# moldyn/Clustering

Hardware: AMD Instinct MI355X
Metric: frame-pairs/s (density pop+nn) (higher is better)
Workload: dtype f32 (Gram form on two fp16 pieces per coordinate on the f16 MFMA pipe, f32 accumulate, as a classifier with a guard band; undecided pairs re-checked in canonical f32)

## Files before the change

clustering_amd/csrc/dc_mfma.hip:

```cpp
#include "dc_mfma_kernels.hpp"
#include "dc_against.hpp"
#include "dc_against_nn.hpp"

#include <algorithm>
#include <cstring>
#include <atomic>
#include <mutex>

#ifndef DC_STEP_MASK
#define DC_STEP_MASK 0xFFFFu
#endif

namespace dc {

namespace {

#include "dc_mfma32.hpp"

__global__ void colsum_kernel(const float* __restrict__ coords, uint32_t n_rows, uint32_t D,
                              double* __restrict__ sums) {
  __shared__ double part[kMaxCols];
  if (threadIdx.x < (uint32_t)kMaxCols) part[threadIdx.x] = 0.0;
  __syncthreads();
  const uint32_t nthreads = gridDim.x * blockDim.x;
// ... 871 lines not shown
    auto env = [](const char* name) -> const char* {
      const char* v = getenv(name);
      return (v && v[0]) ? v : nullptr;
    };
    auto one_of_124 = [](const char* v, int dflt) {
      const int k = v ? atoi(v) : dflt;
      return (k == 1 || k == 2 || k == 4) ? k : dflt;
    };
    SweepSwitches w;
    const char* v;
    if ((v = env("DC_POP_SYM"))) w.pop_sym = v[0] != '0';
    if ((v = env("DC_POP_SHARED"))) w.pop_shared = atoi(v);
    if ((v = env("DC_NN_SHARED"))) w.nn_shared = atoi(v);
    w.waves_per_group = one_of_124(env("DC_WAVES_PER_GROUP"), 0);
    if ((v = env("DC_NN_COOP"))) w.nn_coop = atoi(v);
    if ((v = env("DC_WAVE_TARGET"))) w.wave_target = (uint32_t)atoi(v);
    if ((v = env("DC_SHARE_FLOOR"))) w.share_floor = (uint32_t)atoi(v);
    if ((v = env("DC_POP_COMPONENTS"))) w.components = v[0] != '0';
    w.pop_cell_frames = (v = env("DC_POP_CELL_FRAMES")) ? (float)atof(v) : kPopCellFrames;
    w.nn_cell_frames = (v = env("DC_NN_CELL_FRAMES")) ? (float)atof(v) : kNnCellFrames;
    if ((v = env("DC_NN_FE_BITS"))) w.nn_fe_bits = atoi(v);
    w.mfma32_wpb = (uint32_t)one_of_124(env("DC_MFMA32_WPB"), 1);
    if ((v = env("DC_MFMA32_CHUNKS"))) w.mfma32_chunks = (uint32_t)atoi(v);
    return w;
  }();
  return sw;
}

static float cell_frames(bool nn) { return nn ? sweep_switches().nn_cell_frames : sweep_switches().pop_cell_frames; }
static float nn_cell_frames() { return cell_frames(true); }
// ... 319 lines not shown

static int order_own_queries(const PrunedWs& W, const Layout& L, const QueryPlan& Q, const float* d_coords, uint32_t n_rows,
                             uint32_t n_cols, unsigned fine_bits, uint32_t i_from, uint32_t i_to, hipStream_t stream) {
  char* p = W.p;
  const dim3 blk(256);
  const uint32_t kb_q = std::min<uint32_t>((std::max(Q.n_q, 32u * Q.T_q) + 255) / 256, 1024u);
  hipLaunchKernelGGL(order_key_kernel, dim3(kb_q), blk, 0, stream, d_coords, n_cols, W.hdr, (const uint32_t*)W.comp,
                     (uint32_t)fine_bits, i_from, i_to, W.sort.keys_in, W.sort.vals_in, n_rows, (const float*)nullptr, 0u, W.cnt_tab, 0,
                     W.perm_q, W.tile_comp_q, 32u * Q.T_q);
  hipLaunchKernelGGL(order_meta_kernel, dim3(1), dim3(1024), 0, stream, W.hdr, W.comp, (const uint32_t*)W.cnt_tab, kb_q, W.start_q,
                     W.range_q, W.base_q, Q.n_q, Q.group_rows, 0, 0.0f, n_cols);
  const SortRemap remap{W.start_q, W.base_q, (uint32_t)kMaxComp, W.tile_comp_q};
  if (int rc = W.sort.run(W.perm_q, Q.n_q, stream, fine_bits, &remap)) return rc;
  hipLaunchKernelGGL(order_rows2_kernel, dim3((32 * Q.T_q + 255) / 256), blk, order_rows_smem_set(n_cols), stream, d_coords, n_cols,
                     L.NM, (const uint32_t*)W.perm_q, Q.T_q, (float*)nullptr, (float4*)(p + L.off_box_q), (const float*)nullptr,
                     (float*)nullptr, (uint32_t*)nullptr, (float2*)nullptr, (const uint32_t*)W.tile_comp_q, W.origins, W.hdr,
                     (uint4*)nullptr, 0, (float*)nullptr, (uint4*)(p + L.off_img_q), (float*)(p + L.off_norm_q), 1u,
                     QSeg{1u, 0u, 1u}, (unsigned long long*)nullptr, (uint32_t*)nullptr, 0u);
  return 0;
}

static void pop_pruned_one(const PopPlan& plan, const float* d_coords, uint32_t n_rows, uint32_t n_cols,
                           const QuerySel& qs, const Rad2& rad2, int n_rad, uint32_t* d_pops, void* d_ws,
                           const EdgeSink* sink_in, hipStream_t stream, float r2_scale, bool prep, bool comp_clean) {
  const Layout L = make_layout(n_rows, n_cols);
  const PrunedWs W = pruned_ws(d_ws, L, n_rows);
  char* p = W.p;
  const dim3 blk(256), grid_n((n_rows + 255) / 256);
  const QueryPlan Q = query_plan(qs, n_rows, plan.group_tiles);
  const uint32_t T_r = Q.T_r;
  const float r_max = sqrtf(fmaxf(r2_scale, 0.0f)) * 1.0001f;
// ... 11 lines not shown
  if (prep) {
    const uint32_t cookie = data_cookie(d_coords, n_rows, n_cols);
    if (!comp_clean) (void)hipMemsetAsync(W.comp, 0, sizeof(uint32_t) * kCompWords, stream);
    hipLaunchKernelGGL(fine_mark_kernel, grid_n, blk, 0, stream, d_coords, n_rows, n_cols, (const uint32_t*)W.hdr, r_conn,
                       W.comp);
    hipLaunchKernelGGL(components_kernel, dim3(1), dim3(1024), components_smem(), stream, (const uint32_t*)W.hdr,
                       (const float*)(p + kHdrMeans), n_cols, r_conn, n_rows, kPopCellFrames, fine_bits, W.comp,
                       components_off() ? 1 : 0, r_max, cookie, (const double*)(p + L.fixed_end), cell_frames(false));
    if (order_refs(W, Q, d_coords, n_rows, n_cols, fine_bits, nullptr, 0u, fine_bits, fmaxf(r2_scale, 0.0f), plan.shift_steps,
                   stream))
      return;
    {
      const bool ref_queries = Q.q_mode != kQueryOwnOrder;
      hipLaunchKernelGGL(order_rows2_kernel, dim3((32 * T_r + 255) / 256), blk, order_rows_smem_set(n_cols), stream, d_coords, n_cols,
                         L.NM, (const uint32_t*)W.perm_p, T_r, (float*)(p + L.off_coords_p), (float4*)(p + L.off_box_p),
                         (const float*)nullptr, (float*)nullptr, (uint32_t*)nullptr, (float2*)nullptr, (const uint32_t*)W.tile_comp,
                         W.origins, W.hdr, (uint4*)(p + L.off_img_p), 0, (float*)(p + L.off_norm_p),
                         ref_queries ? (uint4*)(p + L.off_img_q) : (uint4*)nullptr, (float*)nullptr, plan.group_tiles, Q.q_seg,
                         (unsigned long long*)(W.comp + kCompHash), pos_clean ? (uint32_t*)(p + L.off_pq) : (uint32_t*)nullptr, 1u);
    }
    if (sink_in && sink_in->best) {
      hipLaunchKernelGGL(gather_u32_kernel, dim3((32 * T_r + 255) / 256), blk, 0, stream, sink_in->comp,
                         (const uint32_t*)W.perm_p, 32u * T_r, W.sort.keys_in);
      hipLaunchKernelGGL(gather_u32_kernel, dim3((32 * T_r + 255) / 256), blk, 0, stream, sink_in->rank,
                         (const uint32_t*)W.perm_p, 32u * T_r, W.sort.keys_out);
    }
    if (Q.q_mode == kQueryOwnOrder &&
        order_own_queries(W, L, Q, d_coords, n_rows, n_cols, fine_bits, qs.i_from, qs.i_to, stream))
      return;
  }
  const uint32_t n_pos_q = 32u * ((Q.q_mode == kQueryOwnOrder) ? Q.T_q : T_r);
// ... 256 lines not shown
  if (reuse_components) {
  } else {
    hipLaunchKernelGGL(fe_key_kernel, dim3(std::min<uint32_t>(grid_n.x, 256u)), blk, 0, stream, d_fe, n_rows, (uint32_t*)nullptr,
                       (uint32_t*)nullptr, W.hdr);
    if (!comp_clean) (void)hipMemsetAsync(W.comp, 0, sizeof(uint32_t) * kCompWords, stream);
    hipLaunchKernelGGL(fine_mark_kernel, grid_n, blk, 0, stream, d_coords, n_rows, n_cols, (const uint32_t*)W.hdr, r_conn, W.comp);
    hipLaunchKernelGGL(components_kernel, dim3(1), dim3(1024), components_smem(), stream, (const uint32_t*)W.hdr,
                       (const float*)(p + kHdrMeans), n_cols, r_conn, n_rows, kNnCellFrames, fine_bits, W.comp,
                       components_off() ? 1 : 0, 0.0f, cookie, (const double*)(p + L.fixed_end), cell_frames(true));
  }
  if (order_refs(W, Q, d_coords, n_rows, n_cols, fine_bits, d_fe, fe_bits, fine_bits + fe_bits, -1.0f ,
                 0, stream))
    return;
  const float* coords_p = (const float*)(p + L.off_coords_p);
  {
    hipLaunchKernelGGL(order_rows2_kernel, dim3((32 * T_r + 255) / 256), blk, order_rows_smem_set(n_cols), stream, d_coords, n_cols,
                       L.NM, (const uint32_t*)W.perm_p, T_r, (float*)(p + L.off_coords_p), (float4*)(p + L.off_box_p), d_fe,
                       (float*)(p + L.off_fe_s), (uint32_t*)(p + L.off_invpos), (float2*)(p + L.off_ferange_p),
                       (const uint32_t*)W.tile_comp, W.origins, W.hdr, (uint4*)(p + L.off_img_p), 2, (float*)(p + L.off_norm_p),
                       own ? (uint4*)nullptr : (uint4*)(p + L.off_img_q), (float*)nullptr, plan.group_tiles, Q.q_seg,
                       (unsigned long long*)(W.comp + kCompHash), (uint32_t*)nullptr, 0u);
  }
  if (own && order_own_queries(W, L, Q, d_coords, n_rows, n_cols, fine_bits, qs.i_from, qs.i_to, stream))
    return;
  const uint32_t n_pos_q = 32u * (own ? Q.T_q : T_r);
  switch (nm_for((int)n_cols)) {
#define X(SV)                                                                                   \
  case SV:                                                                                      \
    if ((DC_STEP_MASK >> (SV - 1)) & 1u)                                                        \
      nn_pruned_step_##SV(plan, d_coords, n_rows, n_cols, d_fe, d_ws, T_r, n_pos_q, Q.q_mode, Q.q_seg, -1.0f, \
                          d_nn_idx, d_nn_d2, d_hd_idx, d_hd_d2, stream);                        \
    break;
    DC_FOR_EACH_S(X)
// ... 489 lines not shown
```

clustering_amd/csrc/dc_mfma.hpp:

```cpp
#pragma once
#include "dc_common.hpp"

namespace dc {

struct EdgeSink {
  uint2* edges;
  unsigned long long* count;
  unsigned long long capacity;
  const uint32_t* comp;
  const uint32_t* rank;
  unsigned long long* best;
};
enum SinkMode { kSinkNone = 0, kSinkPairs = 1, kSinkMinEdge = 2 };

struct SweepSwitches {
  bool pop_sym = true;
  int pop_shared = -1;
  int nn_shared = -1;
  int waves_per_group = 0;
  int nn_coop = -1;
  uint32_t wave_target = 0;
  uint32_t share_floor = 0;
  bool components = true;
  float pop_cell_frames = 0.0f;
  float nn_cell_frames = 0.0f;
  int nn_fe_bits = -1;
  uint32_t mfma32_wpb = 1;
  uint32_t mfma32_chunks = 0;
};
const SweepSwitches& sweep_switches();

enum PopForm {
  kPopWave,
  kPopWaveSym,
  kPopPairs,
// ... 141 lines not shown
```

clustering_amd/csrc/dc_mfma_kernels.hpp:

```cpp
#pragma once
#include "dc_mfma.hpp"
#include "dc_credit.hpp"

#include <assert.h>
#include <float.h>
#include <math.h>
#include <stdlib.h>

#include <type_traits>

namespace dc {

namespace {

typedef float f32x16 __attribute__((ext_vector_type(16)));
typedef short s16x8 __attribute__((ext_vector_type(8)));

constexpr int kMaxCols = 64;
constexpr int kConstSlots = 2;
constexpr int kPieceGroups = 3;
constexpr int nm_for(int n_cols) { return (kPieceGroups * n_cols + kConstSlots + 15) / 16; }
constexpr int kMaxMfma = nm_for(kMaxCols);
constexpr size_t kHdrBytes = 1024;
constexpr size_t kHdrSums = 256;
// ... 23 lines not shown
constexpr size_t kCompAdj = kCompRange + 2 * kCompRangeStride;
constexpr size_t kCompBox = kCompAdj + 2 * (size_t)kMaxComp;
constexpr size_t kCompBitmap = kCompBox + 4 * (size_t)kMaxComp;
constexpr size_t kCompBitmapWords = (size_t)kCoarseCells * kFineSub * kFineSub / 4;
constexpr size_t kCompBase = kCompBitmap + kCompBitmapWords;
constexpr size_t kCompHash = ((kCompBase + 2 * ((size_t)kMaxComp + 1)) + 1) & ~(size_t)1;
constexpr size_t kCompWords = kCompHash + 2 * 64;

struct Layout {
  uint32_t T, NM;
  uint32_t Tp;
  size_t off_img, off_img_b, off_norm, off_img_s, off_norm_s, off_fe_s, off_perm, off_invpos, off_pq,
      off_keys_in, off_keys_out, off_vals_in,
      off_img_p, off_norm_p, off_perm_p, off_box_p, off_img_q, off_norm_q, off_perm_q, off_box_q,
      off_ferange_p,
      off_coords_p,
      off_merge64,
      off_box_t,
      off_comp,
      off_tile_comp, off_tile_comp_q,
      fixed_end;
};

inline size_t align256(size_t x) { return (x + 255) & ~(size_t)255; }

inline Layout make_layout(size_t n_rows, size_t n_cols) {
  Layout L;
  L.T = (uint32_t)((n_rows + 31) / 32);
  L.NM = (uint32_t)nm_for((int)n_cols);
  L.Tp = L.T + kPadTiles;
  const size_t img_bytes = (size_t)16 * 64 * (size_t)L.Tp * L.NM;
  const size_t row_bytes = align256(sizeof(float) * 32 * (size_t)L.Tp);
  L.off_comp = kHdrBytes;
// ... 6 lines not shown
  L.off_perm = L.off_fe_s + row_bytes;
  L.off_invpos = L.off_perm + row_bytes;
  L.off_pq = L.off_invpos + row_bytes;
  L.off_keys_in = L.off_pq + row_bytes;
  L.off_keys_out = L.off_keys_in + row_bytes;
  L.off_vals_in = L.off_keys_out + row_bytes;
  L.off_img_p = L.off_vals_in + row_bytes;
  L.off_norm_p = align256(L.off_img_p + img_bytes);
  L.off_perm_p = L.off_norm_p + row_bytes;
  L.off_box_p = L.off_perm_p + row_bytes;
  L.off_img_q = align256(L.off_box_p + sizeof(float) * 4 * (size_t)L.Tp);
  L.off_norm_q = align256(L.off_img_q + img_bytes);
  L.off_perm_q = L.off_norm_q + row_bytes;
  L.off_box_q = L.off_perm_q + row_bytes;
  L.off_ferange_p = align256(L.off_box_q + sizeof(float) * 4 * (size_t)L.Tp);
  L.off_coords_p = align256(L.off_ferange_p + sizeof(float) * 2 * (size_t)L.Tp);
  L.off_merge64 = align256(L.off_coords_p + sizeof(float) * 32 * (size_t)L.Tp * n_cols);
  L.off_box_t = align256(L.off_merge64 + sizeof(unsigned long long) * 2 * n_rows);
  L.off_tile_comp = align256(L.off_box_t + sizeof(float) * 4 * ((size_t)L.Tp + L.Tp / 32 + 64));
  L.off_tile_comp_q = align256(L.off_tile_comp + sizeof(uint32_t) * (size_t)L.Tp);
  L.fixed_end = align256(L.off_tile_comp_q + sizeof(uint32_t) * (size_t)L.Tp);
  return L;
}

struct Ptrs {
  const uint32_t* hdr;
  const double* sums;
  const uint4* img;
  const uint4* img_b;
  const float* norms;
  const uint4* img_s;
  const float* norms_s;
  const float* fe_s;
  const uint32_t* perm;
// ... 1555 lines not shown
__device__ __forceinline__ void load_tile_folded(const uint4* __restrict__ img, uint32_t t, int lane, s16x8 (&a)[NM]) {
  const uint4* ip = img + (size_t)t * (NM * 64) + lane;
#pragma unroll
  for (int m = 0; m < NM; ++m) {
    const uint4 v = ip[m * 64];
    a[m] = __builtin_bit_cast(s16x8, v);
  }
}

template <int NM, int TQ, bool COOP = false>
__global__ __launch_bounds__(COOP ? 512 : 256, COOP ? 1 : 2) void nn_pruned_kernel(
    const float* __restrict__ coords, uint32_t n_rows, uint32_t n_cols,
    const float* __restrict__ fe, const uint4* __restrict__ img_r,
    const float* __restrict__ norms_r, const uint32_t* __restrict__ perm_r,
    const float4* __restrict__ box_r, const float4* __restrict__ box_t,
    const float2* __restrict__ ferange_r,
    const float* __restrict__ fe_c, const float* __restrict__ coords_c,
    const uint32_t* __restrict__ invpos_r, uint32_t T,
    const uint4* __restrict__ img_q, const float* __restrict__ norms_q,
    const uint32_t* __restrict__ perm_q, const float4* __restrict__ box_q, uint32_t n_q, QSeg q_seg,
    int full_range, float cell2,
    const uint32_t* __restrict__ hdr, unsigned long long* __restrict__ chain_counter,
    unsigned long long* __restrict__ merge64, uint32_t* __restrict__ nn_idx,
    float* __restrict__ nn_d2, uint32_t* __restrict__ hd_idx, float* __restrict__ hd_d2, CompView CV) {
  extern __shared__ __attribute__((aligned(16))) float nn_dyn_lds[];
  if (hdr[1] != 0) return;
  const int lane = threadIdx.x & 63, h = lane >> 5, c = lane & 31;
  const int wib = threadIdx.x >> 6;
  const uint32_t wpb = blockDim.x >> 6;
  uint32_t* lists_all = reinterpret_cast<uint32_t*>(nn_dyn_lds);
// ... 240 lines not shown
    own_hi = (uint32_t)__builtin_amdgcn_readfirstlane((int)own_hi);
  }
  const float fe_floor = fkey_inv(~hdr[12]);
  auto flush = [&]() {
    nn_wave_flush(cand, qn, qrows, best64, TQ * 32, coords_c, perm_r, n_cols, lane);
    qn = 0;
  };
  uint32_t chains = 0, visited = 0;
  uint32_t chains_on = 0;
  const uint32_t t_lo = comp_lo, t_hi = min(comp_hi, T);
  const uint32_t u_lo = (t_lo > chunk) ? (t_lo - chunk + n_chunks - 1) / n_chunks : 0u;
  const uint32_t U = max((t_hi > chunk) ? (t_hi - chunk + n_chunks - 1) / n_chunks : 0u, u_lo);
  cell2 = comp_cell * comp_cell;
  const uint32_t U_stride = (T + n_chunks - 1) / n_chunks;
  const float dgx = gbox.y - gbox.x, dgy = gbox.w - gbox.z;
  float r2_lo = -1.0f;
  float r2_hi = fmaxf(dgx * dgx + dgy * dgy, cell2);
  if (!(r2_hi > 0.0f)) r2_hi = FLT_MIN;
  for (;;) {
    for (uint32_t base = u_lo; base < U; base += kListCap) {
      uint32_t cnt = 0;
      const uint32_t lim = min(U - base, (uint32_t)kListCap);
      auto tile_of = [&](uint32_t u) { return chunk + u * n_chunks; };
      const float4* box_s = box_t + (size_t)chunk * U_stride;
      float4 rb_next = ((uint32_t)lane < lim) ? box_s[base + lane]
                                              : make_float4(INFINITY, -INFINITY, INFINITY, -INFINITY);
      for (uint32_t k = 0; k < lim; k += 64) {
        const uint32_t t = tile_of(base + k + lane);
        const float4 rb = rb_next;
        if (k + 64 + lane < lim) rb_next = box_s[base + k + 64 + lane];
        bool ok = false;
        if (k + lane < lim) {
          const float g2 = box_gap2(gbox, rb);
          ok = (g2 < r2_hi) & (g2 >= r2_lo);
        }
        const uint64_t m = __builtin_amdgcn_ballot_w64(ok);
        if (ok) list[cnt + __builtin_amdgcn_mbcnt_hi((uint32_t)(m >> 32), __builtin_amdgcn_mbcnt_lo((uint32_t)m, 0))] = t;
        cnt += (uint32_t)__builtin_popcountll(m);
      }
      if (cnt == 0) continue;
      visited += cnt;
      uint32_t cN = 0, cH = 0;
      if constexpr (kNnEarly<NM>) {
        constexpr int kSteps = kListCap / 64;
        uint32_t e[kSteps], cls[kSteps];
        float2 fr[kSteps];
#pragma unroll
        for (int j = 0; j < kSteps; ++j) {
// ... 366 lines not shown
  const uint32_t waves = (tiles + tq - 1) / tq;
  return (waves + 3) / 4;
}

template <int S, SweepMode M>
void pop_dispatch(const SweepArgs& X, uint32_t n_cols, uint32_t i_from, uint32_t i_to, const Rad2& rad2, uint32_t* pops,
                  hipStream_t s) {
  constexpr int kTQ = tq_full_for<S>;
  const dim3 grid(grid_for(i_from, i_to, kTQ)), block(256);
  sweep_timer_mark(0, true, s);
  hipLaunchKernelGGL((pop_mfma_kernel<S, 1, kTQ, M>), grid, block, 0, s, X, n_cols, i_from, i_to, rad2, 1, pops);
  sweep_timer_mark(0, false, s);
}

__global__ void box_by_share_kernel(const float4* __restrict__ box_r, uint32_t T, uint32_t n_chunks,
                                    float4* __restrict__ box_t) {
  const uint32_t t = blockIdx.x * blockDim.x + threadIdx.x;
  if (t >= T) return;
  const uint32_t stride = (T + n_chunks - 1) / n_chunks;
  box_t[(size_t)(t % n_chunks) * stride + t / n_chunks] = box_r[t];
}

struct NnPrunedArgs {
  const uint4* img_r;
  const float* norms_r;
  const uint32_t* perm_r;
  const float4* box_r;
  float4* box_t;
  const float2* ferange_r;
  const float* fe_c;
  const float* coords_c;
  const uint32_t* invpos_r;
  const uint4* img_q;
  const float* norms_q;
  const uint32_t* perm_q;
  const float4* box_q;
  unsigned long long* merge64;
  uint32_t n_q;
  QSeg q_seg;
  int full_range;
  float cell2;
  const uint32_t* tile_comp_q;
  const uint32_t* comp;
// ... 83 lines not shown
  if (sw.share_floor) share_floor = sw.share_floor;
  const uint32_t waves = (tiles + tq - 1) / tq;
  uint32_t r = waves >= target ? 1u : (target + waves - 1) / waves;
  const uint32_t by_share = ref_tiles / share_floor;
  const uint32_t cap = by_share < 64u ? by_share : 64u;
  r = r > cap ? cap : r;
  return r < 1u ? 1u : r;
}

template <class F>
void timed_launch(int kind, hipStream_t s, F&& launch) {
  sweep_timer_mark(kind, true, s);
  launch();
  sweep_timer_mark(kind, false, s);
}
inline void nn_shares_begin(const NnPrunedArgs& A, uint32_t n_rows, uint32_t T, uint32_t n_chunks, hipStream_t s) {
  if (n_chunks > 1)
    hipLaunchKernelGGL(nn_merge_fill_kernel, dim3((2 * n_rows + 255) / 256), dim3(256), 0, s, A.merge64, n_rows);
  hipLaunchKernelGGL(box_by_share_kernel, dim3((T + 255) / 256), dim3(256), 0, s, A.box_r, T, n_chunks, A.box_t);
}
inline void nn_shares_end(const NnPrunedArgs& A, uint32_t n_rows, uint32_t n_chunks, uint32_t group_tiles,
                          uint32_t* nn_idx, float* nn_d2, uint32_t* hd_idx, float* hd_d2, hipStream_t s) {
  if (n_chunks <= 1) return;
  if (A.full_range)
    hipLaunchKernelGGL(nn_merge_unpack_rows_kernel, dim3((n_rows + 255) / 256), dim3(256), 0, s,
                       (const unsigned long long*)A.merge64, A.invpos_r, n_rows, group_tiles, A.q_seg, nn_idx, nn_d2,
                       hd_idx, hd_d2);
  else
    hipLaunchKernelGGL(nn_merge_unpack_kernel, dim3((A.n_q + 255) / 256), dim3(256), 0, s,
                       (const unsigned long long*)A.merge64, A.perm_q, A.n_q, n_rows, group_tiles, A.q_seg, nn_idx,
                       nn_d2, hd_idx, hd_d2);
}

template <int S>
void nn_pruned_dispatch(const NnPlan& pl, const float* coords, uint32_t n_rows, uint32_t n_cols, const float* fe,
                        const NnPrunedArgs& A, uint32_t T, const uint32_t* hdr,
                        unsigned long long* chain_counter, uint32_t* nn_idx, float* nn_d2,
                        uint32_t* hd_idx, float* hd_d2, hipStream_t s) {
  assert(nn_form_built(pl.form, S));
  if (A.n_q == 0) return;
  const CompView CV{A.tile_comp_q, A.comp + kCompRange, 32u * T, A.comp};
  if (pl.form == kNnShared) {
    if constexpr (nn_form_built(kNnShared, S)) {
      constexpr int TQV = tq_wave(S);
      assert(pl.tq == (uint32_t)TQV);
      const uint32_t groups = seg_groups(((A.n_q + 31) / 32 + 4 * TQV - 1) / (4 * TQV), A.q_seg);
      if (groups == 0) return;
      const uint32_t n_chunks = pick_chunks(groups * 4 * TQV, TQV, kNnWaveTarget, T, kNnShareFloor, (size_t)S * 1024 + 128);
      const size_t smem = (size_t)kRing * (S * 64 + kNnRingExtra) * 16 + sizeof(uint32_t) * 4 * (TQV * kQueueCap * 64 + TQV * 32);
      nn_shares_begin(A, n_rows, T, n_chunks, s);
      constexpr int kNbMax = kNnCoarseMax<S>;
      constexpr int kNbMin = (S > 1) ? nn_coarse_for((16 * (S - 1) - kConstSlots) / kPieceGroups + 1) : kNbMax;
      auto launch = [&](auto nb_c) {
        timed_launch(1, s, [&] {
          hipLaunchKernelGGL((nn_shared_kernel<S, TQV, decltype(nb_c)::value>), dim3(grid_x8(groups), n_chunks), dim3(256), smem, s, coords,
                             n_rows, n_cols, fe, A.img_r, A.norms_r, A.perm_r, A.box_r, (const float4*)A.box_t, A.ferange_r, A.fe_c,
                             A.coords_c, A.invpos_r, T, A.img_q, A.norms_q, A.perm_q, A.box_q, A.n_q, A.q_seg, A.full_range, A.cell2,
                             hdr, chain_counter, A.merge64, nn_idx, nn_d2, hd_idx, hd_d2, CV);
        });
      };
      if constexpr (kNbMin != kNbMax) {
        if (nn_coarse_for((int)n_cols) < kNbMax)
          launch(std::integral_constant<int, kNbMin>{});
        else
          launch(std::integral_constant<int, kNbMax>{});
// ... 1 lines not shown
        launch(std::integral_constant<int, kNbMax>{});
      }
      nn_shares_end(A, n_rows, n_chunks, 4u * TQV, nn_idx, nn_d2, hd_idx, hd_d2, s);
    }
    return;
  }
  constexpr int TQV = tq_nn(S);
  assert(pl.tq == (uint32_t)TQV);
  const uint32_t waves = seg_groups(((A.n_q + 31) / 32 + TQV - 1) / TQV, A.q_seg), tiles = waves * TQV;
  if (waves == 0) return;
  uint32_t n_chunks = pick_chunks(tiles, TQV, kNnWaveTargetPerWave, T, kNnShareFloor, (size_t)S * 1024 + 128);
  if (n_chunks >= pl.coop_shares) {
    n_chunks = (n_chunks + kNnCoopWaves - 1) / kNnCoopWaves * kNnCoopWaves;
    const size_t smem_c = sizeof(uint32_t) * (kNnCoopWaves * (kListCap + 2 * kWaveQueue) + 8 * TQV * 32) +
                          sizeof(float) * TQV * 32 * (size_t)n_cols;
    nn_shares_begin(A, n_rows, T, n_chunks, s);
    timed_launch(1, s, [&] {
      hipLaunchKernelGGL((nn_pruned_kernel<S, TQV, true>), dim3(grid_x8(waves), n_chunks / kNnCoopWaves), dim3(64 * kNnCoopWaves), smem_c, s,
                         coords, n_rows, n_cols, fe, A.img_r, A.norms_r, A.perm_r, A.box_r, (const float4*)A.box_t, A.ferange_r,
                         A.fe_c, A.coords_c, A.invpos_r, T, A.img_q, A.norms_q, A.perm_q, A.box_q, A.n_q, A.q_seg,
                         A.full_range, A.cell2, hdr, chain_counter, A.merge64, nn_idx, nn_d2, hd_idx, hd_d2, CV);
    });
  } else {
    const uint32_t wpb = pl.waves;
    const size_t smem = wpb * (sizeof(uint32_t) * kListCap + sizeof(float) * TQV * 32 * (size_t)n_cols +
                               sizeof(uint32_t) * (TQV * kQueueCap * 64 + 2 * TQV * 32));
    nn_shares_begin(A, n_rows, T, n_chunks, s);
    timed_launch(1, s, [&] {
      hipLaunchKernelGGL((nn_pruned_kernel<S, TQV>), dim3(grid_x8((waves + wpb - 1) / wpb), n_chunks), dim3(64 * wpb), smem, s,
                         coords, n_rows, n_cols, fe, A.img_r, A.norms_r, A.perm_r, A.box_r, (const float4*)A.box_t, A.ferange_r,
                         A.fe_c, A.coords_c, A.invpos_r, T, A.img_q, A.norms_q, A.perm_q, A.box_q, A.n_q, A.q_seg,
                         A.full_range, A.cell2, hdr, chain_counter, A.merge64, nn_idx, nn_d2, hd_idx, hd_d2, CV);
    });
  }
  nn_shares_end(A, n_rows, n_chunks, (uint32_t)TQV, nn_idx, nn_d2, hd_idx, hd_d2, s);
}

__global__ void pops_by_frame_kernel(const uint32_t* __restrict__ pops_pos, const uint32_t* __restrict__ perm,
                                     uint32_t n_rows, const uint32_t* __restrict__ hdr, uint32_t* __restrict__ pops) {
  if (hdr[1] != 0) return;
  const uint32_t pos = blockIdx.x * blockDim.x + threadIdx.x;
  if (pos < n_rows && perm[pos] != kInvalidFrame) pops[perm[pos]] = pops_pos[pos];
}

template <int S>
void pop_pruned_dispatch(const PopPlan& pl, const float* coords, uint32_t n_rows, uint32_t n_cols, const Ptrs& P,
// ... 144 lines not shown
```

clustering_amd/csrc/dc_mfma_step.hip:

```cpp
#include "dc_mfma_kernels.hpp"

#ifndef DC_STEP
#error "compile with -DDC_STEP=<MFMAs per tile pair>"
#endif
#define DC_CAT2(a, b) a##b
#define DC_CAT(a, b) DC_CAT2(a, b)

namespace dc {

void DC_CAT(pop_mfma_step_, DC_STEP)(const SweepArgs& X, SweepMode mode, uint32_t n_cols, uint32_t i_from,
                                     uint32_t i_to, const Rad2& rad2, uint32_t* pops, hipStream_t s) {
  (mode == kSelf ? pop_dispatch<DC_STEP, kSelf> : pop_dispatch<DC_STEP, kAgainst>)(X, n_cols, i_from, i_to, rad2, pops,
                                                                                   s);
}

void DC_CAT(pop_pruned_step_, DC_STEP)(const PopPlan& plan, const float* coords, uint32_t n_rows, uint32_t n_cols,
                                       void* d_ws, uint32_t T_ref, uint32_t n_q, int q_mode, QSeg q_seg,
                                       const Rad2& rad2, int n_rad, uint32_t* pops,
                                       const EdgeSink* sink, hipStream_t s, bool pos_clean) {
  const Layout L = make_layout(n_rows, n_cols);
  pop_pruned_dispatch<DC_STEP>(plan, coords, n_rows, n_cols, ws_ptrs(d_ws, L), T_ref, n_q, q_mode, q_seg,
                               rad2, n_rad, pops, (unsigned long long*)((char*)d_ws + 8), sink, s, pos_clean);
}

void DC_CAT(nn_pruned_step_, DC_STEP)(const NnPlan& plan, const float* coords, uint32_t n_rows, uint32_t n_cols,
                                      const float* fe, void* d_ws, uint32_t T_ref, uint32_t n_q, int q_mode,
                                      QSeg q_seg, float cell2, uint32_t* nn_idx, float* nn_d2,
                                      uint32_t* hd_idx, float* hd_d2, hipStream_t s) {
  const Layout L = make_layout(n_rows, n_cols);
  char* p = (char*)d_ws;
  NnPrunedArgs A;
  A.img_r = (const uint4*)(p + L.off_img_p);
  A.norms_r = (const float*)(p + L.off_norm_p);
  A.perm_r = (const uint32_t*)(p + L.off_perm_p);
  A.box_r = (const float4*)(p + L.off_box_p);
  A.box_t = (float4*)(p + L.off_box_t);
  A.ferange_r = (const float2*)(p + L.off_ferange_p);
  A.fe_c = (const float*)(p + L.off_fe_s);
  A.coords_c = (const float*)(p + L.off_coords_p);
  A.invpos_r = (const uint32_t*)(p + L.off_invpos);
  const bool own = q_mode == kQueryOwnOrder;
  A.img_q = (const uint4*)(p + L.off_img_q);
  A.norms_q = own ? (const float*)(p + L.off_norm_q) : A.norms_r;
  A.perm_q = own ? (const uint32_t*)(p + L.off_perm_q) : A.perm_r;
  A.box_q = own ? (const float4*)(p + L.off_box_q) : A.box_r;
  A.q_seg = q_seg;
  A.merge64 = (unsigned long long*)(p + L.off_merge64);
  A.n_q = n_q;
  A.full_range = (q_mode == kQueryAll) ? 1 : 0;
  A.cell2 = cell2;
  A.tile_comp_q = (const uint32_t*)(p + (own ? L.off_tile_comp_q : L.off_tile_comp));
  A.comp = (const uint32_t*)(p + L.off_comp);
// ... 14 lines not shown
```

clustering_amd/csrc/dc_prep.hpp:

```cpp
#pragma once

constexpr float kStatsLimit = 5.0e16f;

constexpr uint32_t kStatsRow = kMaxCols + 3;
constexpr uint32_t kStatsMaxBlocks = 2048;
__global__ __launch_bounds__(256) void stats_kernel(const float* __restrict__ coords, uint32_t n_rows, uint32_t D,
                                                    uint32_t* __restrict__ hdr, uint32_t cookie, double* __restrict__ table) {
  __shared__ double part[kMaxCols];
  __shared__ uint32_t wave_max[4];
  __shared__ unsigned long long fp_part[4];
  if (threadIdx.x < (uint32_t)kMaxCols) part[threadIdx.x] = 0.0;
  __syncthreads();
  const uint32_t nthreads = gridDim.x * blockDim.x;
  const uint32_t used = (nthreads / D) * D;
  const uint32_t id = blockIdx.x * blockDim.x + threadIdx.x;
  const size_t total = (size_t)n_rows * D;
  const uint32_t* w = reinterpret_cast<const uint32_t*>(coords);
  const uint32_t col = id % D;
  double s0 = 0.0, s1 = 0.0, s2 = 0.0, s3 = 0.0;
  uint32_t m_lo = 0, m_hi = 0;
  unsigned long long fp = 0;
  bool bad = false;
  auto take = [&](uint32_t bits, size_t e, double& s) {
    const float v = __uint_as_float(bits);
// ... 485 lines not shown
  for (uint32_t m = 0; m < NM; ++m) {
    const uint32_t* f = src + 8u * m;
    img_out[m * 64u + (uint32_t)lane] = make_uint4(f[0], f[1], f[2], f[3]);
  }
  __builtin_amdgcn_wave_barrier();
}

static inline size_t order_rows_smem(uint32_t n_cols) {
  const uint32_t NM = (uint32_t)nm_for((int)n_cols);
  return sizeof(float) * 256 * (n_cols | 1u) + 4 * (sizeof(unsigned short) * 32 * (16 * NM + 2) + sizeof(float) * n_cols);
}

__global__ __launch_bounds__(256) void order_rows2_kernel(
    const float* __restrict__ coords, uint32_t D, uint32_t NM, const uint32_t* __restrict__ perm, uint32_t T,
    float* __restrict__ coords_o, float4* __restrict__ boxes, const float* __restrict__ fe, float* __restrict__ fe_s,
    uint32_t* __restrict__ invpos, float2* __restrict__ ferange, const uint32_t* __restrict__ tile_comp,
    const float* __restrict__ origins, uint32_t* __restrict__ hdr, uint4* __restrict__ img_a, int a_form,
    float* __restrict__ norms_a, uint4* __restrict__ img_b, float* __restrict__ norms_b, uint32_t grp_tq, QSeg grp,
    unsigned long long* __restrict__ hash_slots, uint32_t* __restrict__ zero_pos, uint32_t zero_planes) {
  extern __shared__ float or_tile[];
  __shared__ uint32_t s_frame[256];
  __shared__ unsigned long long fp_part[4];
  const uint32_t Dp = D | 1u;
  const uint32_t pos0 = blockIdx.x * 256u, pos = pos0 + threadIdx.x, n_pos = 32u * T;
  const uint32_t frame = (pos < n_pos) ? perm[pos] : kInvalidFrame;
  s_frame[threadIdx.x] = frame;
  if (zero_pos && pos < n_pos)
    for (uint32_t z = 0; z < zero_planes; ++z) zero_pos[(size_t)z * n_pos + pos] = 0u;
  __syncthreads();
  const size_t base = (size_t)pos0 * D, total = (size_t)n_pos * D;
  for (uint32_t e0 = threadIdx.x; e0 < 256u * D; e0 += 1024u) {
// ... 34 lines not shown
    }
    fp_publish(in_range ? fp_term(frame, pos) : 0ull, hash_slots + (blockIdx.x & 63u), fp_part);
  }
#pragma unroll
  for (int off = 16; off > 0; off >>= 1) {
    lo0 = fminf(lo0, __shfl_xor(lo0, off, 64));
    hi0 = fmaxf(hi0, __shfl_xor(hi0, off, 64));
    lo1 = fminf(lo1, __shfl_xor(lo1, off, 64));
    hi1 = fmaxf(hi1, __shfl_xor(hi1, off, 64));
    flo = fminf(flo, __shfl_xor(flo, off, 64));
    fhi = fmaxf(fhi, __shfl_xor(fhi, off, 64));
  }
  if ((pos & 31u) == 0 && in_range) {
    boxes[t] = make_float4(lo0, hi0, lo1, hi1);
    if (ferange) ferange[t] = make_float2(flo, fhi);
  }
  const int lane = (int)(threadIdx.x & 63u), wv = (int)(threadIdx.x >> 6);
  unsigned short* lds_img = reinterpret_cast<unsigned short*>(or_tile + 256u * Dp) + (size_t)wv * (32u * img_stride_halves(NM) + 2u * D);
  float* org = reinterpret_cast<float*>(lds_img + 32u * img_stride_halves(NM));
  const Scale sc = load_scale(hdr);
  const float* means = reinterpret_cast<const float*>(reinterpret_cast<const char*>(hdr) + kHdrMeans);
  for (uint32_t tt = 0; tt < 2u; ++tt) {
    const uint32_t lt = 2u * (uint32_t)wv + tt, tile = blockIdx.x * 8u + lt;
    if (tile >= T) break;
    const uint32_t tc = tile_comp[tile];
    const float* o = (tc < (uint32_t)kMaxComp) ? origins + (size_t)tc * kMaxCols : means;
    for (uint32_t k = (uint32_t)lane; k < D; k += 64u) org[k] = o[k];
    __builtin_amdgcn_fence(__ATOMIC_RELEASE, "wavefront");
    __builtin_amdgcn_wave_barrier();
    const float* trows = or_tile + (size_t)lt * 32u * Dp;
// ... 138 lines not shown
```

Measured before the change: 93690 billion.

## Add radial-distance gap bound to prune reference tiles in NN sweep

Each reference tile now records the range of its rows' distances from the component origin in the dimensions beyond the first two. The NN pruning test adds the squared gap between the query group's range and the tile's range to the 2-D box gap, which is a valid lower bound by the triangle inequality. The aim is to reject more reference tiles before the MFMA distance work. It costs an extra double-precision pass per row in order_rows2, plus more workspace and extra loads in the tile scan. The bound is only sound when both sides use the same origin, and the code only turns it on in query-all mode.

```diff
diff --git a/clustering_amd/csrc/dc_mfma.hip b/clustering_amd/csrc/dc_mfma.hip
--- a/clustering_amd/csrc/dc_mfma.hip
+++ b/clustering_amd/csrc/dc_mfma.hip
@@ -909,6 +909,7 @@
     if ((v = env("DC_NN_SHARED"))) w.nn_shared = atoi(v);
     w.waves_per_group = one_of_124(env("DC_WAVES_PER_GROUP"), 0);
     if ((v = env("DC_NN_COOP"))) w.nn_coop = atoi(v);
+    if ((v = env("DC_NN_RHO"))) w.nn_rho = v[0] != '0';
     if ((v = env("DC_WAVE_TARGET"))) w.wave_target = (uint32_t)atoi(v);
     if ((v = env("DC_SHARE_FLOOR"))) w.share_floor = (uint32_t)atoi(v);
     if ((v = env("DC_POP_COMPONENTS"))) w.components = v[0] != '0';
@@ -1258,7 +1259,8 @@
   if (int rc = W.sort.run(W.perm_q, Q.n_q, stream, fine_bits, &remap)) return rc;
   hipLaunchKernelGGL(order_rows2_kernel, dim3((32 * Q.T_q + 255) / 256), blk, order_rows_smem_set(n_cols), stream, d_coords, n_cols,
                      L.NM, (const uint32_t*)W.perm_q, Q.T_q, (float*)nullptr, (float4*)(p + L.off_box_q), (const float*)nullptr,
-                     (float*)nullptr, (uint32_t*)nullptr, (float2*)nullptr, (const uint32_t*)W.tile_comp_q, W.origins, W.hdr,
+                     (float*)nullptr, (uint32_t*)nullptr, (float2*)nullptr, (float2*)nullptr, (const uint32_t*)W.tile_comp_q, W.origins,
+                     W.hdr,
                      (uint4*)nullptr, 0, (float*)nullptr, (uint4*)(p + L.off_img_q), (float*)(p + L.off_norm_q), 1u,
                      QSeg{1u, 0u, 1u}, (unsigned long long*)nullptr, (uint32_t*)nullptr, 0u);
   return 0;
@@ -1300,7 +1302,8 @@
       const bool ref_queries = Q.q_mode != kQueryOwnOrder;
       hipLaunchKernelGGL(order_rows2_kernel, dim3((32 * T_r + 255) / 256), blk, order_rows_smem_set(n_cols), stream, d_coords, n_cols,
                          L.NM, (const uint32_t*)W.perm_p, T_r, (float*)(p + L.off_coords_p), (float4*)(p + L.off_box_p),
-                         (const float*)nullptr, (float*)nullptr, (uint32_t*)nullptr, (float2*)nullptr, (const uint32_t*)W.tile_comp,
+                         (const float*)nullptr, (float*)nullptr, (uint32_t*)nullptr, (float2*)nullptr, (float2*)nullptr,
+                         (const uint32_t*)W.tile_comp,
                          W.origins, W.hdr, (uint4*)(p + L.off_img_p), 0, (float*)(p + L.off_norm_p),
                          ref_queries ? (uint4*)(p + L.off_img_q) : (uint4*)nullptr, (float*)nullptr, plan.group_tiles, Q.q_seg,
                          (unsigned long long*)(W.comp + kCompHash), pos_clean ? (uint32_t*)(p + L.off_pq) : (uint32_t*)nullptr, 1u);
@@ -1587,9 +1590,11 @@
     return;
   const float* coords_p = (const float*)(p + L.off_coords_p);
   {
+    const bool with_rho = !own && sweep_switches().nn_rho;
     hipLaunchKernelGGL(order_rows2_kernel, dim3((32 * T_r + 255) / 256), blk, order_rows_smem_set(n_cols), stream, d_coords, n_cols,
                        L.NM, (const uint32_t*)W.perm_p, T_r, (float*)(p + L.off_coords_p), (float4*)(p + L.off_box_p), d_fe,
                        (float*)(p + L.off_fe_s), (uint32_t*)(p + L.off_invpos), (float2*)(p + L.off_ferange_p),
+                       with_rho ? (float2*)(p + L.off_rhorange_p) : (float2*)nullptr,
                        (const uint32_t*)W.tile_comp, W.origins, W.hdr, (uint4*)(p + L.off_img_p), 2, (float*)(p + L.off_norm_p),
                        own ? (uint4*)nullptr : (uint4*)(p + L.off_img_q), (float*)nullptr, plan.group_tiles, Q.q_seg,
                        (unsigned long long*)(W.comp + kCompHash), (uint32_t*)nullptr, 0u);
diff --git a/clustering_amd/csrc/dc_mfma.hpp b/clustering_amd/csrc/dc_mfma.hpp
--- a/clustering_amd/csrc/dc_mfma.hpp
+++ b/clustering_amd/csrc/dc_mfma.hpp
@@ -19,6 +19,7 @@
   int nn_shared = -1;
   int waves_per_group = 0;
   int nn_coop = -1;
+  bool nn_rho = true;
   uint32_t wave_target = 0;
   uint32_t share_floor = 0;
   bool components = true;
diff --git a/clustering_amd/csrc/dc_mfma_kernels.hpp b/clustering_amd/csrc/dc_mfma_kernels.hpp
--- a/clustering_amd/csrc/dc_mfma_kernels.hpp
+++ b/clustering_amd/csrc/dc_mfma_kernels.hpp
@@ -1,6 +1,7 @@
 #pragma once
 #include "dc_mfma.hpp"
 #include "dc_credit.hpp"
+#include "dc_rho_gap.hpp"
 
 #include <assert.h>
 #include <float.h>
@@ -61,9 +62,11 @@
       off_keys_in, off_keys_out, off_vals_in,
       off_img_p, off_norm_p, off_perm_p, off_box_p, off_img_q, off_norm_q, off_perm_q, off_box_q,
       off_ferange_p,
+      off_rhorange_p,
       off_coords_p,
       off_merge64,
       off_box_t,
+      off_rho_t,
       off_comp,
       off_tile_comp, off_tile_comp_q,
       fixed_end;
@@ -100,10 +103,12 @@
   L.off_perm_q = L.off_norm_q + row_bytes;
   L.off_box_q = L.off_perm_q + row_bytes;
   L.off_ferange_p = align256(L.off_box_q + sizeof(float) * 4 * (size_t)L.Tp);
-  L.off_coords_p = align256(L.off_ferange_p + sizeof(float) * 2 * (size_t)L.Tp);
+  L.off_rhorange_p = align256(L.off_ferange_p + sizeof(float) * 2 * (size_t)L.Tp);
+  L.off_coords_p = align256(L.off_rhorange_p + sizeof(float) * 2 * (size_t)L.Tp);
   L.off_merge64 = align256(L.off_coords_p + sizeof(float) * 32 * (size_t)L.Tp * n_cols);
   L.off_box_t = align256(L.off_merge64 + sizeof(unsigned long long) * 2 * n_rows);
-  L.off_tile_comp = align256(L.off_box_t + sizeof(float) * 4 * ((size_t)L.Tp + L.Tp / 32 + 64));
+  L.off_rho_t = align256(L.off_box_t + sizeof(float) * 4 * ((size_t)L.Tp + L.Tp / 32 + 64));
+  L.off_tile_comp = align256(L.off_rho_t + sizeof(float) * 2 * ((size_t)L.Tp + L.Tp / 32 + 64));
   L.off_tile_comp_q = align256(L.off_tile_comp + sizeof(uint32_t) * (size_t)L.Tp);
   L.fixed_end = align256(L.off_tile_comp_q + sizeof(uint32_t) * (size_t)L.Tp);
   return L;
@@ -1689,6 +1694,7 @@
     const float* __restrict__ fe, const uint4* __restrict__ img_r,
     const float* __restrict__ norms_r, const uint32_t* __restrict__ perm_r,
     const float4* __restrict__ box_r, const float4* __restrict__ box_t,
+    const float2* __restrict__ rho_r, const float2* __restrict__ rho_t,
     const float2* __restrict__ ferange_r,
     const float* __restrict__ fe_c, const float* __restrict__ coords_c,
     const uint32_t* __restrict__ invpos_r, uint32_t T,
@@ -1959,6 +1965,19 @@
   cell2 = comp_cell * comp_cell;
   const uint32_t U_stride = (T + n_chunks - 1) / n_chunks;
   const float dgx = gbox.y - gbox.x, dgy = gbox.w - gbox.z;
+  float grho_lo = 0.0f, grho_hi = 0.0f;
+  if (rho_r) {
+    grho_lo = INFINITY;
+    grho_hi = -INFINITY;
+#pragma unroll
+    for (int qt = 0; qt < TQ; ++qt) {
+      const float2 v = (qt0 + qt < TQT) ? rho_r[qt0 + qt] : make_float2(INFINITY, -INFINITY);
+      grho_lo = fminf(grho_lo, v.x);
+      grho_hi = fmaxf(grho_hi, v.y);
+    }
+    grho_lo = __uint_as_float((uint32_t)__builtin_amdgcn_readfirstlane((int)__float_as_uint(grho_lo)));
+    grho_hi = __uint_as_float((uint32_t)__builtin_amdgcn_readfirstlane((int)__float_as_uint(grho_hi)));
+  }
   float r2_lo = -1.0f;
   float r2_hi = fmaxf(dgx * dgx + dgy * dgy, cell2);
   if (!(r2_hi > 0.0f)) r2_hi = FLT_MIN;
@@ -1970,13 +1989,19 @@
       const float4* box_s = box_t + (size_t)chunk * U_stride;
       float4 rb_next = ((uint32_t)lane < lim) ? box_s[base + lane]
                                               : make_float4(INFINITY, -INFINITY, INFINITY, -INFINITY);
+      const float2* rho_s = rho_t ? rho_t + (size_t)chunk * U_stride : nullptr;
+      float2 rr_next = (rho_s && (uint32_t)lane < lim) ? rho_s[base + lane] : make_float2(0.0f, 0.0f);
       for (uint32_t k = 0; k < lim; k += 64) {
         const uint32_t t = tile_of(base + k + lane);
         const float4 rb = rb_next;
-        if (k + 64 + lane < lim) rb_next = box_s[base + k + 64 + lane];
+        const float2 rr = rr_next;
+        if (k + 64 + lane < lim) {
+          rb_next = box_s[base + k + 64 + lane];
+          if (rho_s) rr_next = rho_s[base + k + 64 + lane];
+        }
         bool ok = false;
         if (k + lane < lim) {
-          const float g2 = box_gap2(gbox, rb);
+          const float g2 = box_gap2(gbox, rb) + rho_gap2(grho_lo, grho_hi, rr.x, rr.y);
           ok = (g2 < r2_hi) & (g2 >= r2_lo);
         }
         const uint64_t m = __builtin_amdgcn_ballot_w64(ok);
@@ -2373,11 +2398,13 @@
 }
 
 __global__ void box_by_share_kernel(const float4* __restrict__ box_r, uint32_t T, uint32_t n_chunks,
-                                    float4* __restrict__ box_t) {
+                                    float4* __restrict__ box_t, const float2* __restrict__ rho_r,
+                                    float2* __restrict__ rho_t) {
   const uint32_t t = blockIdx.x * blockDim.x + threadIdx.x;
   if (t >= T) return;
   const uint32_t stride = (T + n_chunks - 1) / n_chunks;
   box_t[(size_t)(t % n_chunks) * stride + t / n_chunks] = box_r[t];
+  if (rho_r) rho_t[(size_t)(t % n_chunks) * stride + t / n_chunks] = rho_r[t];
 }
 
 struct NnPrunedArgs {
@@ -2386,6 +2413,8 @@
   const uint32_t* perm_r;
   const float4* box_r;
   float4* box_t;
+  const float2* rho_r;
+  float2* rho_t;
   const float2* ferange_r;
   const float* fe_c;
   const float* coords_c;
@@ -2499,10 +2528,11 @@
   launch();
   sweep_timer_mark(kind, false, s);
 }
-inline void nn_shares_begin(const NnPrunedArgs& A, uint32_t n_rows, uint32_t T, uint32_t n_chunks, hipStream_t s) {
+inline void nn_shares_begin(const NnPrunedArgs& A, uint32_t n_rows, uint32_t T, uint32_t n_chunks, bool with_rho, hipStream_t s) {
   if (n_chunks > 1)
     hipLaunchKernelGGL(nn_merge_fill_kernel, dim3((2 * n_rows + 255) / 256), dim3(256), 0, s, A.merge64, n_rows);
-  hipLaunchKernelGGL(box_by_share_kernel, dim3((T + 255) / 256), dim3(256), 0, s, A.box_r, T, n_chunks, A.box_t);
+  hipLaunchKernelGGL(box_by_share_kernel, dim3((T + 255) / 256), dim3(256), 0, s, A.box_r, T, n_chunks, A.box_t,
+                     with_rho ? A.rho_r : (const float2*)nullptr, A.rho_t);
 }
 inline void nn_shares_end(const NnPrunedArgs& A, uint32_t n_rows, uint32_t n_chunks, uint32_t group_tiles,
                           uint32_t* nn_idx, float* nn_d2, uint32_t* hd_idx, float* hd_d2, hipStream_t s) {
@@ -2533,7 +2563,7 @@
       if (groups == 0) return;
       const uint32_t n_chunks = pick_chunks(groups * 4 * TQV, TQV, kNnWaveTarget, T, kNnShareFloor, (size_t)S * 1024 + 128);
       const size_t smem = (size_t)kRing * (S * 64 + kNnRingExtra) * 16 + sizeof(uint32_t) * 4 * (TQV * kQueueCap * 64 + TQV * 32);
-      nn_shares_begin(A, n_rows, T, n_chunks, s);
+      nn_shares_begin(A, n_rows, T, n_chunks, false, s);
       constexpr int kNbMax = kNnCoarseMax<S>;
       constexpr int kNbMin = (S > 1) ? nn_coarse_for((16 * (S - 1) - kConstSlots) / kPieceGroups + 1) : kNbMax;
       auto launch = [&](auto nb_c) {
@@ -2565,22 +2595,22 @@
     n_chunks = (n_chunks + kNnCoopWaves - 1) / kNnCoopWaves * kNnCoopWaves;
     const size_t smem_c = sizeof(uint32_t) * (kNnCoopWaves * (kListCap + 2 * kWaveQueue) + 8 * TQV * 32) +
                           sizeof(float) * TQV * 32 * (size_t)n_cols;
-    nn_shares_begin(A, n_rows, T, n_chunks, s);
+    nn_shares_begin(A, n_rows, T, n_chunks, true, s);
     timed_launch(1, s, [&] {
       hipLaunchKernelGGL((nn_pruned_kernel<S, TQV, true>), dim3(grid_x8(waves), n_chunks / kNnCoopWaves), dim3(64 * kNnCoopWaves), smem_c, s,
-                         coords, n_rows, n_cols, fe, A.img_r, A.norms_r, A.perm_r, A.box_r, (const float4*)A.box_t, A.ferange_r,
-                         A.fe_c, A.coords_c, A.invpos_r, T, A.img_q, A.norms_q, A.perm_q, A.box_q, A.n_q, A.q_seg,
+                         coords, n_rows, n_cols, fe, A.img_r, A.norms_r, A.perm_r, A.box_r, (const float4*)A.box_t, A.rho_r,
+                         (const float2*)(A.rho_r ? A.rho_t : nullptr), A.ferange_r, A.fe_c, A.coords_c, A.invpos_r, T, A.img_q, A.norms_q, A.perm_q, A.box_q, A.n_q, A.q_seg,
                          A.full_range, A.cell2, hdr, chain_counter, A.merge64, nn_idx, nn_d2, hd_idx, hd_d2, CV);
     });
   } else {
     const uint32_t wpb = pl.waves;
     const size_t smem = wpb * (sizeof(uint32_t) * kListCap + sizeof(float) * TQV * 32 * (size_t)n_cols +
                                sizeof(uint32_t) * (TQV * kQueueCap * 64 + 2 * TQV * 32));
-    nn_shares_begin(A, n_rows, T, n_chunks, s);
+    nn_shares_begin(A, n_rows, T, n_chunks, true, s);
     timed_launch(1, s, [&] {
       hipLaunchKernelGGL((nn_pruned_kernel<S, TQV>), dim3(grid_x8((waves + wpb - 1) / wpb), n_chunks), dim3(64 * wpb), smem, s,
-                         coords, n_rows, n_cols, fe, A.img_r, A.norms_r, A.perm_r, A.box_r, (const float4*)A.box_t, A.ferange_r,
-                         A.fe_c, A.coords_c, A.invpos_r, T, A.img_q, A.norms_q, A.perm_q, A.box_q, A.n_q, A.q_seg,
+                         coords, n_rows, n_cols, fe, A.img_r, A.norms_r, A.perm_r, A.box_r, (const float4*)A.box_t, A.rho_r,
+                         (const float2*)(A.rho_r ? A.rho_t : nullptr), A.ferange_r, A.fe_c, A.coords_c, A.invpos_r, T, A.img_q, A.norms_q, A.perm_q, A.box_q, A.n_q, A.q_seg,
                          A.full_range, A.cell2, hdr, chain_counter, A.merge64, nn_idx, nn_d2, hd_idx, hd_d2, CV);
     });
   }
diff --git a/clustering_amd/csrc/dc_mfma_step.hip b/clustering_amd/csrc/dc_mfma_step.hip
--- a/clustering_amd/csrc/dc_mfma_step.hip
+++ b/clustering_amd/csrc/dc_mfma_step.hip
@@ -36,6 +36,9 @@
   A.box_r = (const float4*)(p + L.off_box_p);
   A.box_t = (float4*)(p + L.off_box_t);
   A.ferange_r = (const float2*)(p + L.off_ferange_p);
+  const bool rho = q_mode == kQueryAll && sweep_switches().nn_rho;
+  A.rho_r = rho ? (const float2*)(p + L.off_rhorange_p) : nullptr;
+  A.rho_t = (float2*)(p + L.off_rho_t);
   A.fe_c = (const float*)(p + L.off_fe_s);
   A.coords_c = (const float*)(p + L.off_coords_p);
   A.invpos_r = (const uint32_t*)(p + L.off_invpos);
diff --git a/clustering_amd/csrc/dc_prep.hpp b/clustering_amd/csrc/dc_prep.hpp
--- a/clustering_amd/csrc/dc_prep.hpp
+++ b/clustering_amd/csrc/dc_prep.hpp
@@ -523,7 +523,8 @@
 __global__ __launch_bounds__(256) void order_rows2_kernel(
     const float* __restrict__ coords, uint32_t D, uint32_t NM, const uint32_t* __restrict__ perm, uint32_t T,
     float* __restrict__ coords_o, float4* __restrict__ boxes, const float* __restrict__ fe, float* __restrict__ fe_s,
-    uint32_t* __restrict__ invpos, float2* __restrict__ ferange, const uint32_t* __restrict__ tile_comp,
+    uint32_t* __restrict__ invpos, float2* __restrict__ ferange, float2* __restrict__ rhorange,
+    const uint32_t* __restrict__ tile_comp,
     const float* __restrict__ origins, uint32_t* __restrict__ hdr, uint4* __restrict__ img_a, int a_form,
     float* __restrict__ norms_a, uint4* __restrict__ img_b, float* __restrict__ norms_b, uint32_t grp_tq, QSeg grp,
     unsigned long long* __restrict__ hash_slots, uint32_t* __restrict__ zero_pos, uint32_t zero_planes) {
@@ -588,6 +589,29 @@
   if ((pos & 31u) == 0 && in_range) {
     boxes[t] = make_float4(lo0, hi0, lo1, hi1);
     if (ferange) ferange[t] = make_float2(flo, fhi);
+  }
+  if (rhorange) {
+    float rlo = INFINITY, rhi = -INFINITY;
+    if (live) {
+      const uint32_t tc = tile_comp[t];
+      const float* o = (tc < (uint32_t)kMaxComp) ? origins + (size_t)tc * kMaxCols
+                                                 : reinterpret_cast<const float*>(reinterpret_cast<const char*>(hdr) + kHdrMeans);
+      double r2 = 0.0;
+      for (uint32_t k = 2; k < D; ++k) {
+        const double d = (double)row[k] - (double)o[k];
+        r2 += d * d;
+      }
+      rlo = rhi = (float)sqrt(r2);
+    }
+#pragma unroll
+    for (int off = 16; off > 0; off >>= 1) {
+      rlo = fminf(rlo, __shfl_xor(rlo, off, 64));
+      rhi = fmaxf(rhi, __shfl_xor(rhi, off, 64));
+    }
+    if ((pos & 31u) == 0 && in_range) {
+      if (D > 2) rho_range_widen(rlo, rhi);
+      rhorange[t] = make_float2(rlo, rhi);
+    }
   }
   const int lane = (int)(threadIdx.x & 63u), wv = (int)(threadIdx.x >> 6);
   unsigned short* lds_img = reinterpret_cast<unsigned short*>(or_tile + 256u * Dp) + (size_t)wv * (32u * img_stride_halves(NM) + 2u * D);
diff --git a/clustering_amd/csrc/dc_rho_gap.hpp b/clustering_amd/csrc/dc_rho_gap.hpp
--- /dev/null
+++ b/clustering_amd/csrc/dc_rho_gap.hpp
@@ -0,0 +1,22 @@
+#pragma once
+#include <math.h>
+
+#if defined(__HIPCC__) || defined(__CUDACC__)
+#define DC_RHO_FN __host__ __device__ __forceinline__
+#else
+#define DC_RHO_FN inline
+#endif
+
+DC_RHO_FN void rho_range_widen(float& lo, float& hi) {
+  const float w = hi * 4.76837158203125e-07f + 1.17549435e-38f;
+  if (lo <= hi) {
+    lo = fmaxf(lo - w, 0.0f);
+    hi = hi + w;
+  }
+}
+
+DC_RHO_FN float rho_gap2(float a_lo, float a_hi, float b_lo, float b_hi) {
+  const float g = fmaxf(fmaxf(b_lo - a_hi, a_lo - b_hi), 0.0f);
+  const float p = g * g;
+  return (p >= 7.88860905e-31f) ? p * 0.99999904632568359375f : 0.0f;
+}
diff --git a/scratch/nn_radial_gap_study.py b/scratch/nn_radial_gap_study.py
--- /dev/null
+++ b/scratch/nn_radial_gap_study.py
@@ -0,0 +1,69 @@
+import sys
+import numpy as np
+sys.path.insert(0, '.')
+from clustering_amd.synth import gaussian_blobs
+
+n, d, TQ, GROUPS = 1_000_000, 10, 6, 40
+rng = np.random.default_rng(11)
+c = gaussian_blobs(n, d)
+cent = np.array([(-1.0, -0.5), (0.0, 0.5), (1.0, -0.5)], dtype=np.float32)
+comp = np.argmin(((c[:, None, :2] - cent[None]) ** 2).sum(2), axis=1)
+dens = np.zeros(n)
+for k in range(3):
+    mu = np.zeros(d, dtype=np.float32)
+    mu[:2] = cent[k]
+    dens += np.exp(-((c - mu) ** 2).sum(1) / (2 * 0.08 ** 2))
+fe_analytic = -np.log(dens + 1e-300)
+pops = 1 + rng.poisson(dens / dens.mean() * 7233.0)
+fe_noisy = -np.log(pops / pops.max())
+rho = np.sqrt((c[:, 2:].astype(np.float64) ** 2).sum(1))
+
+
+def order_of(fe, frames_per_cell=128.0):
+    lo, hi = c[:, :2].min(0), c[:, :2].max(0)
+    edge = (np.prod(hi - lo) * frames_per_cell / n / 2.7) ** 0.5
+    idx = np.minimum(((c[:, :2] - lo) / edge).astype(np.int64), 4000)
+    cell = (comp.astype(np.int64) * 4001 + idx[:, 0]) * 4001 + idx[:, 1]
+    fq = ((fe - fe.min()) / (fe.max() - fe.min()) * 65535).astype(np.int64)
+    return np.argsort(cell * 65536 + fq, kind='stable')
+
+
+def study(name, fe):
+    o = order_of(fe)
+    cs, fs, rs, ks = c[o], fe[o], rho[o], comp[o]
+    T = n // 32
+    xy = cs[:T * 32, :2].reshape(T, 32, 2)
+    lo, hi = xy.min(1), xy.max(1)
+    rlo, rhi = rs[:T * 32].reshape(T, 32).min(1), rs[:T * 32].reshape(T, 32).max(1)
+    tk = ks[:T * 32:32]
+    sq = (cs.astype(np.float64) ** 2).sum(1)
+    f2, f2r, gw = [], [], []
+    for g in rng.choice(T // TQ, GROUPS, replace=False):
+        t0 = g * TQ
+        rows = slice(t0 * 32, (t0 + TQ) * 32)
+        q, fq = cs[rows].astype(np.float64), fs[rows]
+        nn, hd = np.full(192, np.inf), np.full(192, np.inf)
+        for b in range(0, n, 100_000):
+            blk = slice(b, min(b + 100_000, n))
+            d2 = (q * q).sum(1)[:, None] + sq[None, blk] - 2.0 * (q @ cs[blk].astype(np.float64).T)
+            own = np.arange(rows.start, rows.stop) - b
+            ok = (own >= 0) & (own < d2.shape[1])
+            d2[np.arange(192)[ok], own[ok]] = np.inf
+            nn = np.minimum(nn, d2.min(1))
+            hd = np.minimum(hd, np.where(fs[None, blk] < fq[:, None], d2, np.inf).min(1))
+        hd = np.where(np.isfinite(hd), hd, 0.0)
+        confirm = max(nn.max(), hd.max())
+        qlo, qhi = lo[t0:t0 + TQ].min(0), hi[t0:t0 + TQ].max(0)
+        gap = np.maximum(0.0, np.maximum(qlo - hi, lo - qhi))
+        g2 = (gap * gap).sum(1)
+        glo, ghi = rlo[t0:t0 + TQ].min(), rhi[t0:t0 + TQ].max()
+        gr = np.where(tk == tk[t0], np.maximum(0.0, np.maximum(rlo - ghi, glo - rhi)), 0.0)
+        f2.append(float((g2 < confirm).mean()))
+        f2r.append(float((g2 + gr * gr < confirm).mean()))
+        gw.append(ghi - glo)
+    print(f"{name:30s} 2-D rings {np.mean(f2):.3f}   2-D + radial gap {np.mean(f2r):.3f}   ratio {np.mean(f2r) / np.mean(f2):.3f}   "
+          f"(tile width in rho: median {np.median(rhi - rlo):.4f}, group width: median {np.median(gw):.3f})", flush=True)
+
+
+study("analytic mixture density", fe_analytic)
+study("Poisson-noised populations", fe_noisy)
```

Result: faster. 95520 billion (median of 6 runs) (+2.0%).
